# bjzhb666/GS-LoRA

Measured on AMD Instinct MI355X. Metric: forgetting-step images/sec, ViT-P8S8 d6 112px r=8, higher is better.
Workload: dtype fp16

## Files before the change

gs-lora_amd/csrc/attention.hip:

```cpp
#include <stdlib.h>

#include <algorithm>
#include <type_traits>

#include "gsl_common.h"

using namespace gsl;
#include "gsl_h16.h"
GSL_OPNS_BEGIN

typedef op16x8_t bf16x8_t;
typedef __attribute__((ext_vector_type(4))) float f32x4_t;

constexpr int HD = 64;
constexpr int KLD = 80;
__device__ __forceinline__ int lds_off(int row, int col) { return row * KLD + col; }

union Frag {
  uint4 u;
  uint2 h[2];
  bf16x8_t v;
};

__device__ __forceinline__ f32x4_t mfma16(const bf16x8_t a, const bf16x8_t b, const f32x4_t c) {
// ... 1229 lines not shown
  long ldi, ko, vo;
};
template <typename T>
__device__ __forceinline__ const T* cls_base(const T* qkv, int b, int h, int Tn, int H, int layout, ClsAddr& a) {
  const long ld3 = 3L * H * HD, ld2 = 2L * H * HD;
  if (layout == 1) { a.ldi = HD; a.ko = (long)Tn * HD; a.vo = 2L * Tn * HD; return qkv + (size_t)(b * H + h) * 3 * Tn * HD; }
  if (layout == 2) { a.ldi = ld2; a.ko = 0; a.vo = (long)H * HD; return qkv + (size_t)b * Tn * ld2 + h * HD; }
  a.ldi = ld3; a.ko = (long)H * HD; a.vo = 2L * H * HD;
  return qkv + (size_t)b * Tn * ld3 + h * HD;
}

template <typename T>
__global__ __launch_bounds__(256) void attn_bwd_cls_kernel(const T* __restrict__ qkv, const T* __restrict__ q_cls, const T* __restrict__ o,
                                                           const T* __restrict__ d_o_cls, const float* __restrict__ lse,
                                                           T* __restrict__ dqkv, T* __restrict__ dq_cls, int Tn, int H, float scale, int hm,
                                                           int cls_compact) {
  GSL_OP16_KERNEL_ENTRY();
  __shared__ float q0[HD], g0[HD], red[32][HD];
  __shared__ float sD;
  const int b = blockIdx.x / H, h = blockIdx.x % H;
  const long ldo = (long)H * HD;
  ClsAddr ad;
  const T* qb = cls_base(qkv, b, h, Tn, H, hm, ad);
  const long ldd = (hm == 2 ? 2L : 3L) * H * HD, dko = (hm == 2) ? 0 : (long)H * HD, dvo = dko + (long)H * HD;
  T* db = dqkv + (size_t)b * Tn * ldd + h * HD;
  const int tid = threadIdx.x;
  if (tid < HD) {
    q0[tid] = Elem<T>::ld(hm == 2 ? q_cls + (size_t)b * ldo + h * HD + tid : qb + tid);
    g0[tid] = Elem<T>::ld(d_o_cls + (size_t)b * ldo + h * HD + tid);
    float v = g0[tid] * Elem<T>::ld(o + (size_t)b * (cls_compact ? 1 : Tn) * ldo + h * HD + tid);
    v = wave_sum(v);
    if (tid == 0) sD = v;
  }
  __syncthreads();
  const float D = sD, l0 = lse[((size_t)b * H + h) * (cls_compact ? 1 : Tn)];
  const int grp = tid >> 3, sub = tid & 7;
  float qs[8], gs[8], dq[8];
#pragma unroll
  for (int i = 0; i < 8; ++i) { qs[i] = q0[sub * 8 + i]; gs[i] = g0[sub * 8 + i]; dq[i] = 0.f; }
  for (int j0 = 0; j0 < Tn; j0 += 32) {
    const int j = j0 + grp;
    const bool live = j < Tn;
    const int jc = live ? j : Tn - 1;
    const T* kr = qb + (size_t)jc * ad.ldi + ad.ko + sub * 8;
    const T* vr = qb + (size_t)jc * ad.ldi + ad.vo + sub * 8;
    float kv[8], vv[8];
    Elem<T>::ld4(kr, kv); Elem<T>::ld4(kr + 4, kv + 4);
    Elem<T>::ld4(vr, vv); Elem<T>::ld4(vr + 4, vv + 4);
    float s = 0.f, dp = 0.f;
#pragma unroll
    for (int i = 0; i < 8; ++i) { s = fmaf(qs[i], kv[i], s); dp = fmaf(gs[i], vv[i], dp); }
#pragma unroll
    for (int sh = 1; sh < 8; sh <<= 1) { s += __shfl_xor(s, sh, 64); dp += __shfl_xor(dp, sh, 64); }
    const float p = expf(s * scale - l0);
    const float ds = p * (dp - D) * scale;
    if (live) {
      float a[8], bb[8];
#pragma unroll
      for (int i = 0; i < 8; ++i) { a[i] = ds * qs[i]; bb[i] = p * gs[i]; dq[i] = fmaf(ds, kv[i], dq[i]); }
      T* dk = db + (size_t)j * ldd + dko + sub * 8;
      T* dv = db + (size_t)j * ldd + dvo + sub * 8;
      Elem<T>::st4(dk, a); Elem<T>::st4(dk + 4, a + 4);
      Elem<T>::st4(dv, bb); Elem<T>::st4(dv + 4, bb + 4);
      if (hm != 2 && j > 0) {
        const float z[4] = {0.f, 0.f, 0.f, 0.f};
        Elem<T>::st4(db + (size_t)j * ldd + sub * 8, z); Elem<T>::st4(db + (size_t)j * ldd + sub * 8 + 4, z);
      }
    }
  }
#pragma unroll
  for (int i = 0; i < 8; ++i) red[grp][sub * 8 + i] = dq[i];
  __syncthreads();
  if (tid < HD) {
    float t = 0.f;
#pragma unroll
    for (int g = 0; g < 32; ++g) t += red[g][tid];
    Elem<T>::st(hm == 2 ? dq_cls + (size_t)b * ldo + h * HD + tid : db + tid, t);
  }
}

template <typename T>
__global__ __launch_bounds__(256) void attn_fwd_cls_kernel(const T* __restrict__ qkv, const T* __restrict__ q_cls, T* __restrict__ o_cls,
                                                           float* __restrict__ lse_cls, int Tn, int H, float scale, int hm) {
  GSL_OP16_KERNEL_ENTRY();
  __shared__ float q0[HD], sc[256], red[32][HD];
  __shared__ float sm[16];
  const int b = blockIdx.x / H, h = blockIdx.x % H;
  const long ldo = (long)H * HD;
  ClsAddr ad;
  const T* qb = cls_base(qkv, b, h, Tn, H, hm, ad);
  const int tid = threadIdx.x;
  if (tid < HD) q0[tid] = Elem<T>::ld(hm == 2 ? q_cls + (size_t)b * ldo + h * HD + tid : qb + tid);
// ... 642 lines not shown
    hipLaunchKernelGGL(attn_fwd_cls_kernel<float>, grid, blk, 0, as_stream(s), (const float*)qkv, (const float*)q_cls, (float*)o_cls, lse_cls, T, H, scale, qkv_layout);
#endif
  else return fail(GSL_ERR_ARG, "gsl_attention_fwd_cls: bad dtype%s %ld", "", dtype);
  return check_launch("gsl_attention_fwd_cls");
}

extern "C" int GSL_ENTRY(gsl_attention_bwd_cls)(const void* qkv, const void* q_cls, const void* o, const void* d_o_cls, const float* lse, void* dqkv,
                                     void* dq_cls, int B, int T, int H, float scale, int dtype, int qkv_layout, int cls_compact,
                                     gsl_stream_t s) {
  GSL_FORWARD_H16(dtype, h16_gsl_attention_bwd_cls(qkv, q_cls, o, d_o_cls, lse, dqkv, dq_cls, B, T, H, scale, dtype, qkv_layout, cls_compact, s));
  GSL_CHECK_ARG(qkv && o && d_o_cls && lse && dqkv && B > 0 && T > 1 && H > 0, "null/size");
  GSL_CHECK_ARG(qkv_layout >= 0 && qkv_layout <= 2 && (qkv_layout != 2 || (q_cls && dq_cls)), "qkv_layout: 0 token-major, 1 head-major, 2 kv + q_cls / dq_cls");
  const dim3 grid(B * H), blk(256);
  if (dtype == GSL_OP16)
    hipLaunchKernelGGL(attn_bwd_cls_kernel<bf16_t>, grid, blk, 0, as_stream(s), (const bf16_t*)qkv, (const bf16_t*)q_cls, (const bf16_t*)o,
                       (const bf16_t*)d_o_cls, lse, (bf16_t*)dqkv, (bf16_t*)dq_cls, T, H, scale, qkv_layout, cls_compact);
#if GSL_HAS_F32
  else if (dtype == GSL_F32)
    hipLaunchKernelGGL(attn_bwd_cls_kernel<float>, grid, blk, 0, as_stream(s), (const float*)qkv, (const float*)q_cls, (const float*)o,
                       (const float*)d_o_cls, lse, (float*)dqkv, (float*)dq_cls, T, H, scale, qkv_layout, cls_compact);
#endif
  else return fail(GSL_ERR_ARG, "gsl_attention_bwd_cls: bad dtype%s %ld", "", dtype);
  return check_launch("gsl_attention_bwd_cls");
}

#ifdef GSL_DEV
static inline int attn_env(const char* name, int dflt) { const char* e = getenv(name); return e ? atoi(e) : dflt; }
static inline unsigned long long* attn_stamps() { const char* sp = getenv("GSL_ATTN_STAMPS"); return sp ? reinterpret_cast<unsigned long long*>(strtoull(sp, nullptr, 0)) : nullptr; }
#else
static inline constexpr int attn_env(const char*, int dflt) { return dflt; }
static inline constexpr unsigned long long* attn_stamps() { return nullptr; }
#endif
static inline int attn_persistent() { return attn_env("GSL_ATTN_PERSISTENT", 1); }
static inline int attn_num_cus() {
  static int n = 0;
  if (!n) {
    int dev = 0; hipDeviceProp_t pr;
    if (hipGetDevice(&dev) == hipSuccess && hipGetDeviceProperties(&pr, dev) == hipSuccess && pr.multiProcessorCount > 0) n = pr.multiProcessorCount;
// ... 129 lines not shown
```

gs-lora_amd/csrc/gsl_h16.h:

```cpp
#pragma once
#include "gsl_common.h"

extern "C" {
int h16_gsl_gemm_nt(const void* A1, int lda1, const void* W1, int ldw1, int K1, const void* A2, int lda2, const void* W2, int ldw2, int K2,
                    int M, int N, int dtype, int epilogue, float alpha, const float* bias, const void* res, const void* aux, void* out,
                    void* out2, int ldo, const float* pos, const float* cls, int T, float p_drop, uint64_t seed, uint32_t site, gsl_stream_t s);
int h16_gsl_gemm_nt_lora(const void* A, int lda, const void* W, int ldw, int K, const void* P, int ldp, const void* Q, int ldq,
                         float lora_scale, void* tout, int ldt, int M, int N, int dtype, int epilogue, const float* bias, const void* res,
                         const void* aux, void* out, void* out2, int ldo, float p_drop, uint64_t seed, uint32_t site, gsl_stream_t s);
int h16_gsl_gemm_nt_lora_mulgrad(const void* A, int lda, const void* W, int ldw, int K, const void* P, int ldp, const void* Q, int ldq,
                                 float lora_scale, void* tout, int ldt, int M, int N, const void* aux, void* out, int ldo, const void* U1,
                                 int ldu1, float* G1, long g1sn, long g1sj, const void* Y2, float* G2, long g2sn, long g2sj, int r,
                                 int accumulate, float* ws, int aux_u8, float p_drop, int dtype, const float* gscale, gsl_stream_t s);
int h16_gsl_attention_fwd(const void* qkv, void* o, float* lse, int B, int T, int H, float scale, int dtype, int qkv_layout, gsl_stream_t s);
int h16_gsl_attention_bwd(const void* qkv, const void* o, const void* d_o, const float* lse, void* dqkv, float* delta_ws, int B, int T,
                          int H, float scale, int dtype, int qkv_layout, gsl_stream_t s);
int h16_gsl_attention_fwd_cls(const void* qkv, const void* q_cls, void* o_cls, float* lse_cls, int B, int T, int H, float scale, int dtype,
                              int qkv_layout, gsl_stream_t s);
int h16_gsl_attention_bwd_cls(const void* qkv, const void* q_cls, const void* o, const void* d_o_cls, const float* lse, void* dqkv,
                              void* dq_cls, int B, int T, int H, float scale, int dtype, int qkv_layout, int cls_compact, gsl_stream_t s);
}

#ifdef GSL_OP_F16
#define GSL_FORWARD_H16(dtype, call)
#define GSL_HAS_F32 0
#else
#define GSL_FORWARD_H16(dtype, call) do { if ((dtype) == GSL_F16) return call; } while (0)
#define GSL_HAS_F32 1
#endif
```

gs-lora_amd/csrc/norm.hip:

```cpp
#include "gsl_common.h"

using namespace gsl;

template <int NPL>
struct RowIO {
  static constexpr int VEC = (NPL % 4 == 0) ? 4 : 1;
  static constexpr int NV = NPL / VEC;
  static __device__ __forceinline__ int idx(int lane, int c, int i) { return (c * 64 + lane) * VEC + i; }
  template <typename T>
  static __device__ __forceinline__ void load(const T* row, int lane, float v[NPL]) {
#pragma unroll
    for (int c = 0; c < NV; ++c) {
      if constexpr (VEC == 4) Elem<T>::ld4(row + (c * 64 + lane) * 4, &v[c * 4]);
      else v[c] = Elem<T>::ld(row + c * 64 + lane);
    }
  }
  template <typename T>
  static __device__ __forceinline__ void store(T* row, int lane, const float v[NPL]) {
#pragma unroll
    for (int c = 0; c < NV; ++c) {
      if constexpr (VEC == 4) Elem<T>::st4(row + (c * 64 + lane) * 4, &v[c * 4]);
      else Elem<T>::st(row + c * 64 + lane, v[c]);
    }
  }
// ... 62 lines not shown
      s2 += gy[i] * xv[i];
    }
    const float c1 = wave_sum(s1) * (1.0f / D), c2 = wave_sum(s2) * (1.0f / D);
#pragma unroll
    for (int i = 0; i < NPL; ++i) gy[i] = rs * (gy[i] - c1 - xv[i] * c2);
    if (dres && (cls_T == 0 || (row % cls_T) == 0)) {
      float r[NPL];
      IO::load(dres + (size_t)(cls_T ? row / cls_T : row) * ios, lane, r);
#pragma unroll
      for (int i = 0; i < NPL; ++i) gy[i] += r[i];
    }
    if (gmax) {
#pragma unroll
      for (int i = 0; i < NPL; ++i) am = fmaxf(am, fabsf(gy[i]));
    }
    IO::store(dx + (size_t)row * (cls_T ? (long)D : ios), lane, gy);
    if (dxb) {
      if (drop.thr) {
#pragma unroll
        for (int c = 0; c < IO::NV; ++c) {
          if constexpr (IO::VEC == 4) {
            float dm[4];
            drop_mul4(drop, (uint64_t)row * drop_row_stride + IO::idx(lane, c, 0), dm);
#pragma unroll
            for (int i = 0; i < 4; ++i) gy[c * 4 + i] *= dm[i];
          } else {
            gy[c] *= drop_mul(drop, (uint64_t)row * drop_row_stride + IO::idx(lane, c, 0));
          }
        }
      }
      IO::store(dxb + (size_t)row * D, lane, gy);
// ... 148 lines not shown
                                 void* y, float* mean, float* rstd, int M, int D, int dtype, int x_dtype, gsl_stream_t s) {
  GSL_CHECK_ARG(x && gamma && beta && mean && rstd && M > 0, "null/size");
  GSL_CHECK_ARG(dtype == GSL_F32 || dtype == GSL_BF16 || dtype == GSL_F16, "dtype");
  GSL_CHECK_ARG(x_dtype == GSL_F32 || ((x_dtype == GSL_BF16 || x_dtype == GSL_F16) && dtype == GSL_BF16) || (x_dtype == GSL_F16 && dtype == GSL_F16),
                "x dtype (a 16-bit stream only in a 16-bit mode; bf16 stream only with bf16 operands)");
  GSL_CHECK_ARG((x_row_stride % 4) == 0, "row stride alignment");
#define CALL(N) ln_fwd_launch<N>(x, x_row_stride, gamma, beta, eps, y, mean, rstd, M, dtype, x_dtype, as_stream(s))
  GSL_DISPATCH_D(D, CALL)
#undef CALL
}

extern "C" int gsl_layernorm_bwd(const void* dy, const void* x, long x_row_stride, const float* gamma, const float* mean,
                                 const float* rstd, const void* dres, void* dx, long io_row_stride, void* dxb, int M, int D,
                                 int dtype, int stream_dtype, int x_dtype, float p_drop, uint64_t seed, uint32_t site,
                                 long drop_row_stride, int dres_cls_T, float* gmax, gsl_stream_t s) {
  GSL_CHECK_ARG(dy && x && gamma && mean && rstd && dx && M > 0, "null/size");
  GSL_CHECK_ARG(dtype == GSL_F32 || dtype == GSL_BF16 || dtype == GSL_F16, "dtype");
  GSL_CHECK_ARG(stream_dtype == GSL_F32 || (stream_dtype == dtype && dtype != GSL_F32), "stream dtype (f32, or the operand format of a 16-bit mode)");
  GSL_CHECK_ARG(x_dtype == GSL_F32 || ((x_dtype == GSL_BF16 || x_dtype == GSL_F16) && dtype == GSL_BF16) || (x_dtype == GSL_F16 && dtype == GSL_F16),
                "x dtype (a 16-bit stream only in a 16-bit mode; bf16 stream only with bf16 operands)");
  GSL_CHECK_ARG((x_row_stride % 4) == 0, "row stride alignment");
  GSL_CHECK_ARG(dres_cls_T >= 0 && (dres_cls_T == 0 || (dres && dres != dx)), "dres_cls_T: compact dres, out of place");
  const DropCfg drop = make_drop(p_drop, seed, site);
  const long ios = io_row_stride > 0 ? io_row_stride : D, drs = drop_row_stride > 0 ? drop_row_stride : D;
  GSL_CHECK_ARG((ios % 4) == 0, "io row stride alignment");
#define CALL(N) ln_bwd_launch<N>(dy, x, x_row_stride, gamma, mean, rstd, dres, dx, ios, dxb, M, dtype, stream_dtype, x_dtype, drop, drs, dres_cls_T, gmax, as_stream(s))
  GSL_DISPATCH_D(D, CALL)
#undef CALL
}

extern "C" int gsl_layernorm_fwd_lora(const void* x, long x_row_stride, const float* gamma, const float* beta, float eps, void* y,
// ... 15 lines not shown
```

gs-lora_amd/gslora_hip/_lib.py:

```python
import ctypes as C
import os

import contextlib

_HERE = os.path.dirname(os.path.abspath(__file__))
LIB_PATH = os.environ.get("GSLORA_HIP_LIB") or os.path.join(_HERE, "libgslora_hip.so")
DEV_LIB_PATH = os.path.join(_HERE, "libgslora_hip_dev.so")

F32, BF16, F16 = 0, 1, 2
EPI_STORE, EPI_BIAS_RES_F32, EPI_BIAS_GELU, EPI_MUL, EPI_PATCH, EPI_STORE_F32, EPI_STORE_QKV_HM, EPI_BIAS_RES_BF16, EPI_PATCH_BF16 = 0, 1, 2, 3, 4, 5, 6, 7, 8
EPI_MUL_G8, EPI_BIAS_GELU_G8, EPI_BIAS_RES_F16, EPI_PATCH_F16, EPI_STORE_LN, EPI_STORE_QKV_HM_LN = 9, 10, 11, 12, 13, 14
VERIF_FLIP_SUM, VERIF_PLAIN = 0, 1
U8_NCHW, U8_NHWC = 0, 1
NORM_SPLIT = 8
SEED_ON_DEVICE = 0x80000000

_vp, _i, _l, _f, _d, _u64, _u32 = C.c_void_p, C.c_int, C.c_long, C.c_float, C.c_double, C.c_uint64, C.c_uint32

SIGNATURES = {
    "gsl_version": [],
    "gsl_last_error": [],
    "gsl_patchify": [_vp, _vp, _i, _i, _i, _i, _i, _i, _vp],
    "gsl_unfold_patches": [_vp, _vp, _i, _i, _i, _i, _i, _i, _i, _i, _i, _vp],
    "gsl_patchify_u8": [_vp, _i, _vp, _vp, _i, _i, _i, _i, _i, _i, _vp],
    "gsl_unfold_patches_u8": [_vp, _i, _vp, _vp, _i, _i, _i, _i, _i, _i, _i, _i, _i, _vp],
    "gsl_gemm_nt": [_vp, _i, _vp, _i, _i, _vp, _i, _vp, _i, _i, _i, _i, _i, _i, _f, _vp, _vp, _vp, _vp, _vp, _i,
                    _vp, _vp, _i, _f, _u64, _u32, _vp],
    "gsl_gemm_nt_lora": [_vp, _i, _vp, _i, _i, _vp, _i, _vp, _i, _f, _vp, _i, _i, _i, _i, _i, _vp, _vp, _vp, _vp, _vp, _i,
                         _f, _u64, _u32, _vp],
    "gsl_gemm_mulgrad_ws_elems": [_i, _i, _i],
    "gsl_gemm_nt_lora_mulgrad": [_vp, _i, _vp, _i, _i, _vp, _i, _vp, _i, _f, _vp, _i, _i, _i, _vp, _vp, _i,
                                 _vp, _i, _vp, _l, _l, _vp, _vp, _l, _l, _i, _i, _vp, _i, _f, _i, _vp, _vp],
    "gsl_layernorm_fwd": [_vp, _l, _vp, _vp, _f, _vp, _vp, _vp, _i, _i, _i, _i, _vp],
    "gsl_layernorm_fwd_lora": [_vp, _l, _vp, _vp, _f, _vp, _vp, _vp, _i, _i, _vp, _i, _f, _vp, _vp],
    "gsl_layernorm_bwd": [_vp, _vp, _l, _vp, _vp, _vp, _vp, _vp, _l, _vp, _i, _i, _i, _i, _i, _f, _u64, _u32, _l, _i, _vp, _vp],
    "gsl_attention_fwd": [_vp, _vp, _vp, _i, _i, _i, _f, _i, _i, _vp],
    "gsl_attention_bwd": [_vp, _vp, _vp, _vp, _vp, _vp, _i, _i, _i, _f, _i, _i, _vp],
    "gsl_attention_fwd_cls": [_vp, _vp, _vp, _vp, _i, _i, _i, _f, _i, _i, _vp],
    "gsl_attention_bwd_cls": [_vp, _vp, _vp, _vp, _vp, _vp, _vp, _i, _i, _i, _f, _i, _i, _i, _vp],
    "gsl_lora_grad_ws_elems": [_i, _i, _i],
    "gsl_lora_grad": [_vp, _l, _vp, _i, _vp, _l, _l, _i, _i, _i, _i, _i, _vp, _vp, _vp],
    "gsl_lora_grad_batch_ws_elems": [_vp, _i],
    "gsl_lora_grad_batch": [_vp, _i, _vp, _i, _vp, _vp],
    "gsl_cosface_prep": [_vp, _vp, _i, _i, _vp],
    "gsl_head_fwd": [_vp, _i, _i, _vp, _vp, _f, _vp, _vp, _vp, _vp, _vp, _vp, _i, _i, _i, _f, _f, _vp, _i, _i, _vp],
    "gsl_head_bwd": [_vp, _vp, _vp, _i, _i, _vp, _vp, _vp, _vp, _vp, _vp, _vp, _i, _i, _i, _f, _i, _i, _f, _u64, _u32, _i, _i, _i, _vp, _vp, _i, _vp],
    "gsl_head_fwd_margin": [_vp, _i, _i, _vp, _vp, _f, _vp, _vp, _vp, _vp, _vp, _vp, _i, _i, _i, _f, _f, _vp, _i, _i, _i, _d, _i, _vp, _vp],
    "gsl_head_bwd_margin": [_vp, _vp, _vp, _i, _i, _vp, _vp, _vp, _vp, _vp, _vp, _vp, _i, _i, _i, _f, _i, _i, _f, _u64, _u32, _i, _i, _i, _vp,
                            _vp, _i, _i, _d, _i, _vp, _vp, _vp],
    "gsl_ce_fwd": [_vp, _vp, _vp, _vp, _i, _i, _vp],
    "gsl_ce_bwd": [_vp, _vp, _vp, _f, _vp, _i, _i, _i, _vp],
    "gsl_proto_kl_fwd": [_vp, _vp, _vp, _vp, _vp, _i, _i, _i, _vp],
    "gsl_loss_combine": [_vp, _vp, _vp, _vp, _vp, _vp, _vp, _f, _f, _f, _f, _f, _f, _f, _f, _vp, _vp, _vp, _vp],
    "gsl_loss_combine_pack": [_vp, _vp, _i, _f, _f, _f, _f, _f, _f, _vp, _vp, _vp, _vp],
# ... 77 lines not shown
```

gs-lora_amd/gslora_hip/ops.py:

```python
import ctypes

import torch

from . import _lib as L

ATTN_MAX_T = 1025


def check_num_tokens(model, T):
    if T > ATTN_MAX_T:
        raise NotImplementedError(f"{model}: this geometry gives {T} tokens per image; the gs-lora_amd attention kernels take at most "
                                  f"{ATTN_MAX_T} (GSL_ATTN_MAX_T: a 32 x 32 patch grid plus the cls token)")


DT = {torch.float32: L.F32, torch.bfloat16: L.BF16, torch.float16: L.F16}


def _p(t):
    return None if t is None else t.data_ptr()


def _stream():
    return torch.cuda.current_stream().cuda_stream

# ... 213 lines not shown
def layernorm_fwd_lora(x, row_stride, M, D, gamma, beta, eps, P, alpha, pad=64):
    _need(x, gamma, beta, P)
    if x.dtype != torch.bfloat16 or P.dtype != torch.bfloat16 or P.shape[0] < 16 or P.shape[1] != D or pad != 64:
        raise ValueError("layernorm_fwd_lora: bf16 x, P [>= 16, D] bf16, 64-column u")
    y = torch.empty(M, D, device=x.device, dtype=torch.bfloat16)
    u = torch.empty(M, pad, device=x.device, dtype=torch.bfloat16)
    mean = torch.empty(M, device=x.device, dtype=torch.float32)
    rstd = torch.empty(M, device=x.device, dtype=torch.float32)
    L.check(L.load().gsl_layernorm_fwd_lora(_p(x), row_stride, _p(gamma), _p(beta), float(eps), _p(y), _p(mean), _p(rstd), M, D,
                                            _p(P), P.stride(0), float(alpha), _p(u), _stream()), "gsl_layernorm_fwd_lora")
    return y, mean, rstd, u


@_profiled("ln_bwd", lambda dy, *a, **k: (dy.shape[0], dy.shape[1], 0, 0))
def layernorm_bwd(dy, x, row_stride, gamma, mean, rstd, dres, want_copy=True, p_drop=0.0, seed=0, site=0, dx=None,
                  io_row_stride=0, drop_row_stride=0, dres_cls_T=0, gmax=None):
    _need(dy, x, gamma, mean, rstd)
    M, D = dy.shape
    sdt = dx.dtype if dx is not None else (dres.dtype if dres is not None else torch.float32)
    own_dx = dx is None
    if dx is None:
        _need(dres)
        dx = torch.empty(M, D, device=dy.device, dtype=sdt)
    elif dres is not None and dres.dtype != dx.dtype:
        raise RuntimeError("layernorm_bwd: dres and dx must share one dtype")
    alias = bool(want_copy) and float(p_drop) == 0.0 and sdt == dy.dtype and own_dx and not io_row_stride
    dxb = torch.empty(M, D, device=dy.device, dtype=dy.dtype) if (want_copy and not alias) else None
    L.check(L.load().gsl_layernorm_bwd(_p(dy), _p(x), row_stride, _p(gamma), _p(mean), _p(rstd), _p(dres), _p(dx),
                                       int(io_row_stride), _p(dxb), M, D, code(dy.dtype), code(sdt), code(x.dtype), float(p_drop),
                                       int(seed), int(site), int(drop_row_stride), int(dres_cls_T), _p(gmax), _stream()), "gsl_layernorm_bwd")
    return dx, (dx if alias else dxb)


@_profiled("attn_fwd", lambda qkv, B, T, H, *a, **k: (B * T, H * 64, T, H))
# ... 23 lines not shown
    L.check(L.load().gsl_attention_fwd_cls(_p(qkv), _p(q_cls), _p(o), _p(lse), B, T, H, float(scale), code(qkv.dtype), int(layout),
                                           _stream()), "gsl_attention_fwd_cls")
    return o, lse


def attention_bwd_cls(qkv, o, d_o_cls, lse, B, T, H, scale, layout=0, q_cls=None):
    _need(qkv, o, d_o_cls, lse, q_cls)
    nw = 2 if layout == 2 else 3
    dqkv = torch.empty(B * T, nw * H * 64, device=qkv.device, dtype=qkv.dtype)
    dq = torch.empty(B, H * 64, device=qkv.device, dtype=qkv.dtype) if layout == 2 else None
    compact = o.shape[0] == B and lse.dim() == 2
    L.check(L.load().gsl_attention_bwd_cls(_p(qkv), _p(q_cls), _p(o), _p(d_o_cls), _p(lse), _p(dqkv), _p(dq), B, T, H, float(scale),
                                           code(qkv.dtype), int(layout), 1 if compact else 0, _stream()), "gsl_attention_bwd_cls")
    return (dqkv, dq) if layout == 2 else dqkv




def lora_grad(Y, U, G, gsn, gsj, r, accumulate=True, gscale=None):
    if not (Y.is_cuda and U.is_cuda and Y.stride(1) == 1 and U.stride(1) == 1):
        raise RuntimeError("lora_grad: operands must be CUDA tensors with unit column stride")
    M, N = Y.shape
    lib = L.load()
    need = lib.gsl_lora_grad_ws_elems(M, N, r)
    ws = _workspace((Y.device.index,), need, Y.device, floor=1 << 22)
    L.check(lib.gsl_lora_grad(_p(Y), Y.stride(0), _p(U), U.stride(0), G.data_ptr(), gsn, gsj, M, N, r, code(Y.dtype),
                              1 if accumulate else 0, _p(ws), _p(gscale), _stream()), "gsl_lora_grad")


class _LgradDesc(ctypes.Structure):
# ... 432 lines not shown
```

gs-lora_amd/gslora_hip/vit_runner.py:

```python
import os

import torch

from . import _lib as L
from . import ops

PADK = 64
OP16 = (torch.bfloat16, torch.float16)
SITE_EMB = 1_000_000
GRAD_STREAM_BF16 = os.environ.get("GSLORA_GRAD_STREAM", "bf16").lower() != "f32"
FWD_STREAM = os.environ.get("GSLORA_FWD_STREAM", "f16").lower()
if FWD_STREAM not in ("f16", "bf16", "f32"):
    raise ValueError(f"GSLORA_FWD_STREAM must be f16, bf16 or f32, not {FWD_STREAM!r}")
GP8 = os.environ.get("GSLORA_GP8", "1") != "0"

FUSE_LORA_GRAD = True
TAIL_CLS = True
QSPLIT = True
INK_MIN_ROWS = 8192
LN1_FOLD = os.environ.get("GSLORA_LN1_FOLD", "1") != "0"
GRAD_TARGET_EXP = int(os.environ.get("GSLORA_GRAD_TARGET_EXP", "0"))
if GRAD_TARGET_EXP and not 4 <= GRAD_TARGET_EXP <= 15:
    raise ValueError(f"GSLORA_GRAD_TARGET_EXP={GRAD_TARGET_EXP}: 0 (default) or 4 .. 15")
INK_SMALL = True
LGRAD_BATCH_MAX_ROWS = 1 << 30
LN_LORA = False
QKV_HEAD_MAJOR = True


class BlockSpec:
    __slots__ = ("ln1", "qkv_w", "qkv_b", "out", "ln2", "l1", "l2", "qkv_lora")

    def __init__(self, ln1, qkv_w, qkv_b, out, ln2, l1, l2, qkv_lora=None):
# ... 529 lines not shown
            del dxn2
            d_o = torch.empty(dx1b.shape[0], c.H * 64, device=c.dev, dtype=c.dt)
            ops.gemm_nt(dx1b, self.wT(f"wo{i}", blk.out.weight, c.dt), d_o)
            if c.attn_site:
                dqkv = self._bwd_attention(c, st, d_o, sparse)
                del d_o, dx1b
                dxn1 = self._bwd_qkv_lora(c, i, blk, st, dqkv)
                del dqkv
                if dxn1 is None:
                    break
            else:
                dxn1 = self._bwd_qkv_frozen(c, i, blk, st, d_o, sparse)
                del d_o, dx1b
            dx, dxb = ops.layernorm_bwd(dxn1, st["x"], c.D, blk.ln1.weight.detach(), st["mean1"], st["rstd1"], dx1,
                                        p_drop=c.p_drop, seed=c.seed, site=(4 * (i - 1) + 2) | c.sflag,
                                        dres_cls_T=c.T if sparse else 0, gmax=c.gmax)
            saved["layers"][i] = None
        if not c.attn_site and not torch.cuda.is_current_stream_capturing():
            self.build_pack_tables(c.dt)

    def _bwd_head(self, c, saved, dlogits, demb):
        sp, dt = c.sp, c.dt
        if dlogits is not None:
            dlogits = dlogits.contiguous().float()
        if demb is not None:
            demb = demb.contiguous().float()
        if dlogits is not None and saved["Wn"] is None:
            raise RuntimeError("backward through logits requires a forward with labels")
        c.gscale = self._loss_scale_state(saved["x_last"].device) if dt == torch.float16 else None
        self._guard_on = c.gscale is not None
        c.gmax = c.gscale[2:] if c.gscale is not None else None
# ... 94 lines not shown
    def _bwd_ln2(self, c, i, blk, st, dxn2, dx, gather):
        gamma, kw = blk.ln2.weight.detach(), dict(p_drop=c.p_drop, seed=c.seed, site=(4 * i) | c.sflag, gmax=c.gmax)
        if gather:
            return ops.layernorm_bwd(dxn2, st["x1"], c.T * c.D, gamma, _cls_rows(c, st["mean2"].view(-1, 1), 1).view(-1),
                                     _cls_rows(c, st["rstd2"].view(-1, 1), 1).view(-1), dx, drop_row_stride=c.T * c.D, **kw)
        return ops.layernorm_bwd(dxn2, st["x1"], c.D, gamma, st["mean2"], st["rstd2"], dx, **kw)

    def _bwd_attention(self, c, st, d_o, sparse):
        if sparse:
            return ops.attention_bwd_cls(st["qkv"], st["o"], d_o, st["lse"], c.B, c.T, c.H, c.sp.attn_scale, layout=st["qkv_hm"], q_cls=st["q_cls"])
        return ops.attention_bwd(st["qkv"], st["o"], d_o, st["lse"], c.B, c.T, c.H, c.sp.attn_scale, layout=st["qkv_hm"])

    def _bwd_qkv_frozen(self, c, i, blk, st, d_o, sparse):
        dt, D, inner = c.dt, c.D, c.H * 64
        dxn1 = torch.empty(c.M, D, device=c.dev, dtype=dt)
        dqkv = self._bwd_attention(c, st, d_o, sparse)
        wt = self.wT(f"qkv{i}", blk.qkv_w, dt)
        if st["q_cls"] is None:
            ops.gemm_nt(dqkv, wt, dxn1)
        else:
            dkv, dq_cls = dqkv
            ops.gemm_nt(dkv, wt[:, inner:], dxn1)
            rows = dxn1.view(c.B, c.T * D)[:, :D]
            ops.gemm_nt(dq_cls, wt[:, :inner], rows, epilogue=_res_epilogue(dt), bias=self._zeros(D, c.dev), res=rows)
        return dxn1

    def _bwd_qkv_lora(self, c, i, blk, st, dqkv):
        dt, D, r, ml = c.dt, c.D, c.r, blk.qkv_lora
        qo = self.qkv_lora_ops(i, ml, dt)
        v = torch.empty(c.M, PADK, device=c.dev, dtype=dt)
        ops.gemm_nt(dqkv, qo["BblkT"], v, alpha=c.s_lora)
        ng, inner = len(ml.enable_lora), c.H * 64
# ... 11 lines not shown
```

include/gslora_hip.h:

```cpp
#ifndef GSLORA_HIP_H
#define GSLORA_HIP_H

#include <stdint.h>

#ifdef __cplusplus
extern "C" {
#endif

#define GSL_API __attribute__((visibility("default")))

typedef void* gsl_stream_t;

enum gsl_dtype { GSL_F32 = 0, GSL_BF16 = 1, GSL_F16 = 2 };

enum gsl_status {
  GSL_OK = 0,
  GSL_ERR_ARG = -1,
  GSL_ERR_LAUNCH = -2,
  GSL_ERR_UNSUPPORTED = -3
};

enum gsl_epilogue {
  GSL_EPI_STORE = 0,
  GSL_EPI_BIAS_RES_F32 = 1,
// ... 54 lines not shown
GSL_API int gsl_layernorm_fwd_lora(const void* x, long x_row_stride, const float* gamma, const float* beta, float eps, void* y,
                           float* mean, float* rstd, int M, int D, const void* P, int ldp, float alpha, void* u, gsl_stream_t s);
GSL_API int gsl_layernorm_bwd(const void* dy, const void* x, long x_row_stride, const float* gamma,
                      const float* mean, const float* rstd, const void* dres,
                      void* dx, long io_row_stride, void* dxb, int M, int D, int dtype, int stream_dtype, int x_dtype,
                      float p_drop, uint64_t seed, uint32_t site, long drop_row_stride, int dres_cls_T, float* gmax, gsl_stream_t s);

#define GSL_ATTN_MAX_T 1025
GSL_API int gsl_attention_fwd(const void* qkv, void* o, float* lse, int B, int T, int H, float scale, int dtype, int qkv_layout, gsl_stream_t s);
GSL_API int gsl_attention_bwd(const void* qkv, const void* o, const void* d_o, const float* lse, void* dqkv,
                      float* delta_ws, int B, int T, int H, float scale, int dtype, int qkv_layout, gsl_stream_t s);
GSL_API int gsl_attention_fwd_cls(const void* qkv, const void* q_cls, void* o_cls, float* lse_cls, int B, int T, int H, float scale,
                                  int dtype, int qkv_layout, gsl_stream_t s);
GSL_API int gsl_attention_bwd_cls(const void* qkv, const void* q_cls, const void* o, const void* d_o_cls, const float* lse, void* dqkv,
                                  void* dq_cls, int B, int T, int H, float scale, int dtype, int qkv_layout, int cls_compact, gsl_stream_t s);

GSL_API long gsl_lora_grad_ws_elems(int M, int N, int r);
GSL_API int gsl_lora_grad(const void* Y, long ldy, const void* U, int ldu, float* G, long gsn, long gsj,
                  int M, int N, int r, int dtype, int accumulate, float* ws, const float* gscale, gsl_stream_t s);
typedef struct gsl_lgrad_desc {
  const void* Y; long ldy; const void* U; int ldu; int M; int N; int r; int accumulate; int pad_; float* G; long gsn, gsj;
} gsl_lgrad_desc;
GSL_API long gsl_lora_grad_batch_ws_elems(const gsl_lgrad_desc* descs, int n);
GSL_API int gsl_lora_grad_batch(const gsl_lgrad_desc* descs, int n, float* ws, int dtype, const float* gscale, gsl_stream_t s);


GSL_API int gsl_cosface_prep(const float* W, float* Wn, int C, int D, gsl_stream_t s);
GSL_API int gsl_head_fwd(const void* x, int x_dtype, int T, const float* gamma, const float* beta, float eps,
                 const float* Wn, const int64_t* label, float* emb, float* mean, float* rstd,
                 float* logits, int B, int D, int C, float cos_s, float cos_m,
// ... 96 lines not shown
```

Baseline: 45160.

## Add rank-structured CLS dKV backward path and skip dead first-layer dx store

Adds an alternative backward for the CLS-only attention site. It stores per-token scalar coefficients (ds, p), projects q_cls, d_o_cls and dq_cls through the frozen QKV weight once per image, then expands dx as a low-rank combination, which avoids the full dqkv tensor and its GEMM. That path is gated behind CLS_DKV_RANK, which defaults to False. The change also lets layernorm_bwd skip writing dx (keeping only the operand copy) for the first layer when no attention site needs it, removing one dead store of M×D; that part is on by default.

New measurement: 45290 (median of 6 runs). Within noise of the previous version (+0.3%).

```diff
diff --git a/gs-lora_amd/csrc/attention.hip b/gs-lora_amd/csrc/attention.hip
--- a/gs-lora_amd/csrc/attention.hip
+++ b/gs-lora_amd/csrc/attention.hip
@@ -1267,7 +1267,7 @@
 __global__ __launch_bounds__(256) void attn_bwd_cls_kernel(const T* __restrict__ qkv, const T* __restrict__ q_cls, const T* __restrict__ o,
                                                            const T* __restrict__ d_o_cls, const float* __restrict__ lse,
                                                            T* __restrict__ dqkv, T* __restrict__ dq_cls, int Tn, int H, float scale, int hm,
-                                                           int cls_compact) {
+                                                           int cls_compact, float* __restrict__ coef) {
   GSL_OP16_KERNEL_ENTRY();
   __shared__ float q0[HD], g0[HD], red[32][HD];
   __shared__ float sD;
@@ -1276,7 +1276,7 @@
   ClsAddr ad;
   const T* qb = cls_base(qkv, b, h, Tn, H, hm, ad);
   const long ldd = (hm == 2 ? 2L : 3L) * H * HD, dko = (hm == 2) ? 0 : (long)H * HD, dvo = dko + (long)H * HD;
-  T* db = dqkv + (size_t)b * Tn * ldd + h * HD;
+  T* db = dqkv ? dqkv + (size_t)b * Tn * ldd + h * HD : nullptr;
   const int tid = threadIdx.x;
   if (tid < HD) {
     q0[tid] = Elem<T>::ld(hm == 2 ? q_cls + (size_t)b * ldo + h * HD + tid : qb + tid);
@@ -1307,7 +1307,14 @@
     for (int sh = 1; sh < 8; sh <<= 1) { s += __shfl_xor(s, sh, 64); dp += __shfl_xor(dp, sh, 64); }
     const float p = expf(s * scale - l0);
     const float ds = p * (dp - D) * scale;
-    if (live) {
+    if (live && coef) {
+#pragma unroll
+      for (int i = 0; i < 8; ++i) dq[i] = fmaf(ds, kv[i], dq[i]);
+      if (sub == 0) {
+        float* cr = coef + ((size_t)b * Tn + j) * 2 * H + h;
+        cr[0] = ds; cr[H] = p;
+      }
+    } else if (live) {
       float a[8], bb[8];
 #pragma unroll
       for (int i = 0; i < 8; ++i) { a[i] = ds * qs[i]; bb[i] = p * gs[i]; dq[i] = fmaf(ds, kv[i], dq[i]); }
@@ -1329,6 +1336,94 @@
 #pragma unroll
     for (int g = 0; g < 32; ++g) t += red[g][tid];
     Elem<T>::st(hm == 2 ? dq_cls + (size_t)b * ldo + h * HD + tid : db + tid, t);
+  }
+}
+
+constexpr int RK_IMG = 64;
+template <typename T>
+__global__ __launch_bounds__(256) void cls_rank_r_kernel(const T* __restrict__ q_cls, const T* __restrict__ d_o_cls, const T* __restrict__ dq_cls,
+                                                         const T* __restrict__ wt, long ldw, float* __restrict__ R, int B, int H, int D, int JR) {
+  GSL_OP16_KERNEL_ENTRY();
+  __shared__ float Ws[HD * (HD + 1)];
+  __shared__ __attribute__((aligned(16))) float Vs[RK_IMG * HD];
+  const int ncb = D / HD, hh = blockIdx.x / ncb, d0 = (blockIdx.x % ncb) * HD, b0 = blockIdx.y * RK_IMG;
+  const int tid = threadIdx.x;
+  const long ldo = (long)H * HD;
+  const T* vsrc = (hh < H ? q_cls + hh * HD : hh < 2 * H ? d_o_cls + (hh - H) * HD : dq_cls + (hh - 2 * H) * HD);
+  const int wc = (hh < 2 * H ? hh + H : hh - 2 * H) * HD;
+#pragma unroll
+  for (int it = 0; it < 4; ++it) {
+    const int qd = tid + it * 256, c = qd >> 4, e4 = (qd & 15) * 4;
+    float w4[4], v4[4] = {0.f, 0.f, 0.f, 0.f};
+    Elem<T>::ld4(wt + (size_t)(d0 + c) * ldw + wc + e4, w4);
+    if (b0 + c < B) Elem<T>::ld4(vsrc + (size_t)(b0 + c) * ldo + e4, v4);
+#pragma unroll
+    for (int i = 0; i < 4; ++i) { Ws[c * (HD + 1) + e4 + i] = w4[i]; Vs[c * HD + e4 + i] = v4[i]; }
+  }
+  __syncthreads();
+  const int c = tid & 63, g = tid >> 6;
+  float w[HD];
+#pragma unroll
+  for (int e = 0; e < HD; ++e) w[e] = Ws[c * (HD + 1) + e];
+  for (int ii = g; ii < RK_IMG && b0 + ii < B; ii += 4) {
+    float acc[4] = {0.f, 0.f, 0.f, 0.f};
+#pragma unroll
+    for (int e4 = 0; e4 < HD / 4; ++e4) {
+      const float4 v = *reinterpret_cast<const float4*>(&Vs[ii * HD + e4 * 4]);
+      float& a = acc[e4 >> 2];
+      a = fmaf(v.x, w[e4 * 4], a); a = fmaf(v.y, w[e4 * 4 + 1], a);
+      a = fmaf(v.z, w[e4 * 4 + 2], a); a = fmaf(v.w, w[e4 * 4 + 3], a);
+    }
+    R[((size_t)(b0 + ii) * JR + hh) * D + d0 + c] = (acc[0] + acc[1]) + (acc[2] + acc[3]);
+  }
+}
+
+constexpr int RK_TC = 256;
+template <typename T, int NJ>
+__global__ __launch_bounds__(256) void cls_rank_expand_kernel(const float* __restrict__ coef, const float* __restrict__ R,
+                                                              T* __restrict__ dx, int Tn, int J, int JR, int D) {
+  GSL_OP16_KERNEL_ENTRY();
+  __shared__ __attribute__((aligned(16))) float cs[RK_TC * NJ];
+  const int b = blockIdx.x, tid = threadIdx.x;
+  const int qr = D >> 2, q = tid % qr, r0 = tid / qr, k = blockDim.x / qr;
+  gsl_f32x2 r[NJ][2];
+#pragma unroll
+  for (int j = 0; j < NJ; ++j) {
+    float4 t = make_float4(0.f, 0.f, 0.f, 0.f);
+    if (j < J) t = *reinterpret_cast<const float4*>(R + ((size_t)b * JR + j) * D + q * 4);
+    r[j][0] = gsl_f32x2{t.x, t.y}; r[j][1] = gsl_f32x2{t.z, t.w};
+  }
+  float4 e = make_float4(0.f, 0.f, 0.f, 0.f);
+  for (int j = J; j < JR; ++j) {
+    const float4 t = *reinterpret_cast<const float4*>(R + ((size_t)b * JR + j) * D + q * 4);
+    e.x += t.x; e.y += t.y; e.z += t.z; e.w += t.w;
+  }
+  for (int t0 = 0; t0 < Tn; t0 += RK_TC) {
+    const int nt = min(RK_TC, Tn - t0);
+    const float* src = coef + ((size_t)b * Tn + t0) * J;
+    if (t0) __syncthreads();
+    for (int i = tid; i < nt * NJ; i += blockDim.x) {
+      const int t = i / NJ, j = i % NJ;
+      cs[i] = j < J ? src[t * J + j] : 0.f;
+    }
+    __syncthreads();
+    for (int t = r0; t < nt; t += k) {
+      gsl_f32x2 a0 = {0.f, 0.f}, a1 = {0.f, 0.f};
+#pragma unroll
+      for (int j4 = 0; j4 < NJ / 4; ++j4) {
+        const float4 c4 = *reinterpret_cast<const float4*>(&cs[t * NJ + j4 * 4]);
+        const float cj[4] = {c4.x, c4.y, c4.z, c4.w};
+#pragma unroll
+        for (int i = 0; i < 4; ++i) {
+          const gsl_f32x2 cc = {cj[i], cj[i]};
+          a0 = __builtin_elementwise_fma(cc, r[j4 * 4 + i][0], a0);
+          a1 = __builtin_elementwise_fma(cc, r[j4 * 4 + i][1], a1);
+        }
+      }
+      float out[4] = {a0[0], a0[1], a1[0], a1[1]};
+      if (t0 + t == 0) { out[0] += e.x; out[1] += e.y; out[2] += e.z; out[3] += e.w; }
+      Elem<T>::st4(dx + ((size_t)b * Tn + t0 + t) * D + q * 4, out);
+    }
   }
 }
 
@@ -2001,14 +2096,78 @@
   const dim3 grid(B * H), blk(256);
   if (dtype == GSL_OP16)
     hipLaunchKernelGGL(attn_bwd_cls_kernel<bf16_t>, grid, blk, 0, as_stream(s), (const bf16_t*)qkv, (const bf16_t*)q_cls, (const bf16_t*)o,
-                       (const bf16_t*)d_o_cls, lse, (bf16_t*)dqkv, (bf16_t*)dq_cls, T, H, scale, qkv_layout, cls_compact);
+                       (const bf16_t*)d_o_cls, lse, (bf16_t*)dqkv, (bf16_t*)dq_cls, T, H, scale, qkv_layout, cls_compact, (float*)nullptr);
 #if GSL_HAS_F32
   else if (dtype == GSL_F32)
     hipLaunchKernelGGL(attn_bwd_cls_kernel<float>, grid, blk, 0, as_stream(s), (const float*)qkv, (const float*)q_cls, (const float*)o,
-                       (const float*)d_o_cls, lse, (float*)dqkv, (float*)dq_cls, T, H, scale, qkv_layout, cls_compact);
+                       (const float*)d_o_cls, lse, (float*)dqkv, (float*)dq_cls, T, H, scale, qkv_layout, cls_compact, (float*)nullptr);
 #endif
   else return fail(GSL_ERR_ARG, "gsl_attention_bwd_cls: bad dtype%s %ld", "", dtype);
   return check_launch("gsl_attention_bwd_cls");
+}
+
+extern "C" int GSL_ENTRY(gsl_attention_bwd_cls_coef)(const void* kv, const void* q_cls, const void* o, const void* d_o_cls, const float* lse,
+                                                     float* coef, void* dq_cls, int B, int T, int H, float scale, int dtype, int cls_compact,
+                                                     gsl_stream_t s) {
+  GSL_FORWARD_H16(dtype, h16_gsl_attention_bwd_cls_coef(kv, q_cls, o, d_o_cls, lse, coef, dq_cls, B, T, H, scale, dtype, cls_compact, s));
+  GSL_CHECK_ARG(kv && q_cls && o && d_o_cls && lse && coef && dq_cls && B > 0 && T > 1 && H > 0, "null/size");
+  const dim3 grid(B * H), blk(256);
+  if (dtype == GSL_OP16)
+    hipLaunchKernelGGL(attn_bwd_cls_kernel<bf16_t>, grid, blk, 0, as_stream(s), (const bf16_t*)kv, (const bf16_t*)q_cls, (const bf16_t*)o,
+                       (const bf16_t*)d_o_cls, lse, (bf16_t*)nullptr, (bf16_t*)dq_cls, T, H, scale, 2, cls_compact, coef);
+#if GSL_HAS_F32
+  else if (dtype == GSL_F32)
+    hipLaunchKernelGGL(attn_bwd_cls_kernel<float>, grid, blk, 0, as_stream(s), (const float*)kv, (const float*)q_cls, (const float*)o,
+                       (const float*)d_o_cls, lse, (float*)nullptr, (float*)dq_cls, T, H, scale, 2, cls_compact, coef);
+#endif
+  else return fail(GSL_ERR_ARG, "gsl_attention_bwd_cls_coef: bad dtype%s %ld", "", dtype);
+  return check_launch("gsl_attention_bwd_cls_coef");
+}
+
+extern "C" int GSL_ENTRY(gsl_cls_rank_r)(const void* q_cls, const void* d_o_cls, const void* dq_cls, const void* wt, long ldw, float* R, int B, int H,
+                                         int D, int dtype, gsl_stream_t s) {
+  GSL_FORWARD_H16(dtype, h16_gsl_cls_rank_r(q_cls, d_o_cls, dq_cls, wt, ldw, R, B, H, D, dtype, s));
+  GSL_CHECK_ARG(q_cls && d_o_cls && wt && R && B > 0 && H > 0 && D > 0, "null/size");
+  GSL_CHECK_ARG(D % HD == 0 && ldw >= 3L * H * HD && ldw % 4 == 0, "D % 64 == 0, ldw >= 3*H*64, rows 4-element aligned");
+  const int JR = (dq_cls ? 3 : 2) * H;
+  const dim3 grid(JR * (D / HD), (B + RK_IMG - 1) / RK_IMG), blk(256);
+  GSL_CHECK_ARG(grid.y <= 65535u, "B <= 65535 * 64");
+  if (dtype == GSL_OP16)
+    hipLaunchKernelGGL(cls_rank_r_kernel<bf16_t>, grid, blk, 0, as_stream(s), (const bf16_t*)q_cls, (const bf16_t*)d_o_cls, (const bf16_t*)dq_cls,
+                       (const bf16_t*)wt, ldw, R, B, H, D, JR);
+#if GSL_HAS_F32
+  else if (dtype == GSL_F32)
+    hipLaunchKernelGGL(cls_rank_r_kernel<float>, grid, blk, 0, as_stream(s), (const float*)q_cls, (const float*)d_o_cls, (const float*)dq_cls,
+                       (const float*)wt, ldw, R, B, H, D, JR);
+#endif
+  else return fail(GSL_ERR_ARG, "gsl_cls_rank_r: bad dtype%s %ld", "", dtype);
+  return check_launch("gsl_cls_rank_r");
+}
+
+template <typename T>
+static int cls_rank_expand_launch(const float* coef, const float* R, void* dx, int B, int Tn, int J, int JR, int D, hipStream_t st) {
+  const int qr = D / 4, k = std::max(1, 256 / qr);
+  const dim3 grid(B), blk(k * qr);
+#define GSL_RKX(NJ) hipLaunchKernelGGL((cls_rank_expand_kernel<T, NJ>), grid, blk, 0, st, coef, R, (T*)dx, Tn, J, JR, D)
+  if (J <= 8) GSL_RKX(8);
+  else if (J <= 16) GSL_RKX(16);
+  else if (J <= 24) GSL_RKX(24);
+  else GSL_RKX(32);
+#undef GSL_RKX
+  return check_launch("gsl_cls_rank_expand");
+}
+
+extern "C" int GSL_ENTRY(gsl_cls_rank_expand)(const float* coef, const float* R, int r_rows, void* dx, int B, int T, int H, int D, int dtype,
+                                              gsl_stream_t s) {
+  GSL_FORWARD_H16(dtype, h16_gsl_cls_rank_expand(coef, R, r_rows, dx, B, T, H, D, dtype, s));
+  GSL_CHECK_ARG(coef && R && dx && B > 0 && T > 0 && H > 0, "null/size");
+  GSL_CHECK_ARG(r_rows == 2 * H || r_rows == 3 * H, "r_rows: 2*H, or 3*H with the Rq rows");
+  GSL_CHECK_ARG(2 * H <= 32 && D > 0 && D % 64 == 0 && D <= 1024, "2*H <= 32, D % 64 == 0, D <= 1024");
+  if (dtype == GSL_OP16) return cls_rank_expand_launch<bf16_t>(coef, R, dx, B, T, 2 * H, r_rows, D, as_stream(s));
+#if GSL_HAS_F32
+  if (dtype == GSL_F32) return cls_rank_expand_launch<float>(coef, R, dx, B, T, 2 * H, r_rows, D, as_stream(s));
+#endif
+  return fail(GSL_ERR_ARG, "gsl_cls_rank_expand: bad dtype%s %ld", "", dtype);
 }
 
 #ifdef GSL_DEV
diff --git a/gs-lora_amd/csrc/gsl_h16.h b/gs-lora_amd/csrc/gsl_h16.h
--- a/gs-lora_amd/csrc/gsl_h16.h
+++ b/gs-lora_amd/csrc/gsl_h16.h
@@ -19,6 +19,11 @@
                               int qkv_layout, gsl_stream_t s);
 int h16_gsl_attention_bwd_cls(const void* qkv, const void* q_cls, const void* o, const void* d_o_cls, const float* lse, void* dqkv,
                               void* dq_cls, int B, int T, int H, float scale, int dtype, int qkv_layout, int cls_compact, gsl_stream_t s);
+int h16_gsl_attention_bwd_cls_coef(const void* kv, const void* q_cls, const void* o, const void* d_o_cls, const float* lse, float* coef,
+                                   void* dq_cls, int B, int T, int H, float scale, int dtype, int cls_compact, gsl_stream_t s);
+int h16_gsl_cls_rank_r(const void* q_cls, const void* d_o_cls, const void* dq_cls, const void* wt, long ldw, float* R, int B, int H, int D, int dtype,
+                       gsl_stream_t s);
+int h16_gsl_cls_rank_expand(const float* coef, const float* R, int r_rows, void* dx, int B, int T, int H, int D, int dtype, gsl_stream_t s);
 }
 
 #ifdef GSL_OP_F16
diff --git a/gs-lora_amd/csrc/norm.hip b/gs-lora_amd/csrc/norm.hip
--- a/gs-lora_amd/csrc/norm.hip
+++ b/gs-lora_amd/csrc/norm.hip
@@ -100,7 +100,7 @@
 #pragma unroll
       for (int i = 0; i < NPL; ++i) am = fmaxf(am, fabsf(gy[i]));
     }
-    IO::store(dx + (size_t)row * (cls_T ? (long)D : ios), lane, gy);
+    if (dx) IO::store(dx + (size_t)row * (cls_T ? (long)D : ios), lane, gy);
     if (dxb) {
       if (drop.thr) {
 #pragma unroll
@@ -279,7 +279,7 @@
                                  const float* rstd, const void* dres, void* dx, long io_row_stride, void* dxb, int M, int D,
                                  int dtype, int stream_dtype, int x_dtype, float p_drop, uint64_t seed, uint32_t site,
                                  long drop_row_stride, int dres_cls_T, float* gmax, gsl_stream_t s) {
-  GSL_CHECK_ARG(dy && x && gamma && mean && rstd && dx && M > 0, "null/size");
+  GSL_CHECK_ARG(dy && x && gamma && mean && rstd && (dx || dxb) && M > 0, "null/size (dx may be NULL only with a dxb)");
   GSL_CHECK_ARG(dtype == GSL_F32 || dtype == GSL_BF16 || dtype == GSL_F16, "dtype");
   GSL_CHECK_ARG(stream_dtype == GSL_F32 || (stream_dtype == dtype && dtype != GSL_F32), "stream dtype (f32, or the operand format of a 16-bit mode)");
   GSL_CHECK_ARG(x_dtype == GSL_F32 || ((x_dtype == GSL_BF16 || x_dtype == GSL_F16) && dtype == GSL_BF16) || (x_dtype == GSL_F16 && dtype == GSL_F16),
diff --git a/gs-lora_amd/gslora_hip/_lib.py b/gs-lora_amd/gslora_hip/_lib.py
--- a/gs-lora_amd/gslora_hip/_lib.py
+++ b/gs-lora_amd/gslora_hip/_lib.py
@@ -38,6 +38,9 @@
     "gsl_attention_bwd": [_vp, _vp, _vp, _vp, _vp, _vp, _i, _i, _i, _f, _i, _i, _vp],
     "gsl_attention_fwd_cls": [_vp, _vp, _vp, _vp, _i, _i, _i, _f, _i, _i, _vp],
     "gsl_attention_bwd_cls": [_vp, _vp, _vp, _vp, _vp, _vp, _vp, _i, _i, _i, _f, _i, _i, _i, _vp],
+    "gsl_attention_bwd_cls_coef": [_vp, _vp, _vp, _vp, _vp, _vp, _vp, _i, _i, _i, _f, _i, _i, _vp],
+    "gsl_cls_rank_r": [_vp, _vp, _vp, _vp, _l, _vp, _i, _i, _i, _i, _vp],
+    "gsl_cls_rank_expand": [_vp, _vp, _i, _vp, _i, _i, _i, _i, _i, _vp],
     "gsl_lora_grad_ws_elems": [_i, _i, _i],
     "gsl_lora_grad": [_vp, _l, _vp, _i, _vp, _l, _l, _i, _i, _i, _i, _i, _vp, _vp, _vp],
     "gsl_lora_grad_batch_ws_elems": [_vp, _i],
diff --git a/gs-lora_amd/gslora_hip/ops.py b/gs-lora_amd/gslora_hip/ops.py
--- a/gs-lora_amd/gslora_hip/ops.py
+++ b/gs-lora_amd/gslora_hip/ops.py
@@ -251,10 +251,19 @@
 
 @_profiled("ln_bwd", lambda dy, *a, **k: (dy.shape[0], dy.shape[1], 0, 0))
 def layernorm_bwd(dy, x, row_stride, gamma, mean, rstd, dres, want_copy=True, p_drop=0.0, seed=0, site=0, dx=None,
-                  io_row_stride=0, drop_row_stride=0, dres_cls_T=0, gmax=None):
+                  io_row_stride=0, drop_row_stride=0, dres_cls_T=0, gmax=None, want_dx=True):
     _need(dy, x, gamma, mean, rstd)
     M, D = dy.shape
     sdt = dx.dtype if dx is not None else (dres.dtype if dres is not None else torch.float32)
+    if not want_dx:
+        if dx is not None or not want_copy:
+            raise RuntimeError("layernorm_bwd: want_dx=False takes no dx buffer and needs the operand copy")
+        _need(dres)
+        dxb = torch.empty(M, D, device=dy.device, dtype=dy.dtype)
+        L.check(L.load().gsl_layernorm_bwd(_p(dy), _p(x), row_stride, _p(gamma), _p(mean), _p(rstd), _p(dres), None,
+                                           int(io_row_stride), _p(dxb), M, D, code(dy.dtype), code(sdt), code(x.dtype), float(p_drop),
+                                           int(seed), int(site), int(drop_row_stride), int(dres_cls_T), _p(gmax), _stream()), "gsl_layernorm_bwd")
+        return None, dxb
     own_dx = dx is None
     if dx is None:
         _need(dres)
@@ -308,6 +317,34 @@
                                            code(qkv.dtype), int(layout), 1 if compact else 0, _stream()), "gsl_attention_bwd_cls")
     return (dqkv, dq) if layout == 2 else dqkv
 
+
+def attention_bwd_cls_coef(kv, o, d_o_cls, lse, B, T, H, scale, q_cls):
+    _need(kv, o, d_o_cls, lse, q_cls)
+    coef = torch.empty(B * T, 2 * H, device=kv.device, dtype=torch.float32)
+    dq = torch.empty(B, H * 64, device=kv.device, dtype=kv.dtype)
+    compact = o.shape[0] == B and lse.dim() == 2
+    L.check(L.load().gsl_attention_bwd_cls_coef(_p(kv), _p(q_cls), _p(o), _p(d_o_cls), _p(lse), _p(coef), _p(dq), B, T, H, float(scale),
+                                                code(kv.dtype), 1 if compact else 0, _stream()), "gsl_attention_bwd_cls_coef")
+    return coef, dq
+
+
+def cls_rank_r(q_cls, d_o_cls, wt, H, dq_cls=None):
+    _need(q_cls, d_o_cls, dq_cls, wt)
+    B, D = q_cls.shape[0], wt.shape[0]
+    if wt.shape[1] != 3 * H * 64:
+        raise RuntimeError(f"cls_rank_r: wt {tuple(wt.shape)} is not [D, 3*{H}*64]")
+    R = torch.empty(B, (2 if dq_cls is None else 3) * H, D, device=q_cls.device, dtype=torch.float32)
+    L.check(L.load().gsl_cls_rank_r(_p(q_cls), _p(d_o_cls), _p(dq_cls), _p(wt), wt.stride(0), _p(R), B, H, D, code(q_cls.dtype), _stream()),
+            "gsl_cls_rank_r")
+    return R
+
+
+def cls_rank_expand(coef, R, out, T):
+    _need(coef, R, out)
+    B, JR, D = R.shape
+    H = coef.shape[1] // 2
+    L.check(L.load().gsl_cls_rank_expand(_p(coef), _p(R), JR, _p(out), B, T, H, D, code(out.dtype), _stream()), "gsl_cls_rank_expand")
+    return out
 
 
 
diff --git a/gs-lora_amd/gslora_hip/vit_runner.py b/gs-lora_amd/gslora_hip/vit_runner.py
--- a/gs-lora_amd/gslora_hip/vit_runner.py
+++ b/gs-lora_amd/gslora_hip/vit_runner.py
@@ -17,6 +17,8 @@
 FUSE_LORA_GRAD = True
 TAIL_CLS = True
 QSPLIT = True
+CLS_DKV_RANK = False
+SKIP_DEAD_DX = True
 INK_MIN_ROWS = 8192
 LN1_FOLD = os.environ.get("GSLORA_LN1_FOLD", "1") != "0"
 GRAD_TARGET_EXP = int(os.environ.get("GSLORA_GRAD_TARGET_EXP", "0"))
@@ -576,7 +578,8 @@
                 del d_o, dx1b
             dx, dxb = ops.layernorm_bwd(dxn1, st["x"], c.D, blk.ln1.weight.detach(), st["mean1"], st["rstd1"], dx1,
                                         p_drop=c.p_drop, seed=c.seed, site=(4 * (i - 1) + 2) | c.sflag,
-                                        dres_cls_T=c.T if sparse else 0, gmax=c.gmax)
+                                        dres_cls_T=c.T if sparse else 0, gmax=c.gmax,
+                                        want_dx=not (SKIP_DEAD_DX and i == 1 and not c.attn_site))
             saved["layers"][i] = None
         if not c.attn_site and not torch.cuda.is_current_stream_capturing():
             self.build_pack_tables(c.dt)
@@ -701,8 +704,12 @@
     def _bwd_qkv_frozen(self, c, i, blk, st, d_o, sparse):
         dt, D, inner = c.dt, c.D, c.H * 64
         dxn1 = torch.empty(c.M, D, device=c.dev, dtype=dt)
+        wt = self.wT(f"qkv{i}", blk.qkv_w, dt)
+        if sparse and st["q_cls"] is not None and CLS_DKV_RANK:
+            coef, dq_cls = ops.attention_bwd_cls_coef(st["qkv"], st["o"], d_o, st["lse"], c.B, c.T, c.H, c.sp.attn_scale, st["q_cls"])
+            R = ops.cls_rank_r(st["q_cls"], d_o, wt, c.H, dq_cls=dq_cls)
+            return ops.cls_rank_expand(coef, R, dxn1, c.T)
         dqkv = self._bwd_attention(c, st, d_o, sparse)
-        wt = self.wT(f"qkv{i}", blk.qkv_w, dt)
         if st["q_cls"] is None:
             ops.gemm_nt(dqkv, wt, dxn1)
         else:
diff --git a/include/gslora_hip.h b/include/gslora_hip.h
--- a/include/gslora_hip.h
+++ b/include/gslora_hip.h
@@ -92,6 +92,12 @@
                                   int dtype, int qkv_layout, gsl_stream_t s);
 GSL_API int gsl_attention_bwd_cls(const void* qkv, const void* q_cls, const void* o, const void* d_o_cls, const float* lse, void* dqkv,
                                   void* dq_cls, int B, int T, int H, float scale, int dtype, int qkv_layout, int cls_compact, gsl_stream_t s);
+GSL_API int gsl_attention_bwd_cls_coef(const void* kv, const void* q_cls, const void* o, const void* d_o_cls, const float* lse, float* coef,
+                                       void* dq_cls, int B, int T, int H, float scale, int dtype, int cls_compact, gsl_stream_t s);
+GSL_API int gsl_cls_rank_r(const void* q_cls, const void* d_o_cls, const void* dq_cls, const void* wt, long ldw, float* R, int B, int H, int D,
+                           int dtype, gsl_stream_t s);
+GSL_API int gsl_cls_rank_expand(const float* coef, const float* R, int r_rows, void* dx, int B, int T, int H, int D, int dtype,
+                                gsl_stream_t s);
 
 GSL_API long gsl_lora_grad_ws_elems(int M, int N, int r);
 GSL_API int gsl_lora_grad(const void* Y, long ldy, const void* U, int ldu, float* G, long gsn, long gsj,
```
